# asalimil/Nonlinear-MPC-for-collision-free-and-deadlock-free-navigation-of-multiple-nonholonomic-mobile-robots

Hardware: AMD Instinct MI355X
Metric: NMPC solves/sec (batched swarms), N_robots=6, N=20 (higher is better)
Workload: dtype f64

## Files before the change

nonlinear-mpc-for-collision-free-and-deadlock-free-navigation-of-multiple-nonholonomic-mobile-robots_amd/csrc/nmpc_solve_col.hip:

```cpp
#include "nmpc_solve_common.h"

namespace nmpc {

__device__ __forceinline__ double lane_read(double v, int lane)
{
    return __hiloint2double(__builtin_amdgcn_readlane(__double2hiint(v), lane), __builtin_amdgcn_readlane(__double2loint(v), lane));
}
#ifndef NMPC_COL_GB
#define NMPC_COL_GB ((M_ == 6) ? (NX + 2) / 2 : NX + 1)
#endif
#ifndef NMPC_FW_PD
#define NMPC_FW_PD ((M_ <= 6) ? 2 : 1)
#endif
#ifndef NMPC_FW_FAKE
#define NMPC_FW_FAKE 0
#endif
#ifndef NMPC_COL_DPP
#define NMPC_COL_DPP 1
#endif
#ifndef NMPC_COL_WAVES_SMALL
#define NMPC_COL_WAVES_SMALL 1
#endif
#ifndef NMPC_COL_WAVES_MID
#define NMPC_COL_WAVES_MID 1
#endif
#ifndef NMPC_COL_WAVES_FOUR
#define NMPC_COL_WAVES_FOUR 2
#endif
#ifndef NMPC_COL_WAVES_LAT
#define NMPC_COL_WAVES_LAT 2
#endif
#ifndef NMPC_COL_DUMMY_ST
#define NMPC_COL_DUMMY_ST (NU - 1)
#endif
#ifndef NMPC_FUSE_DPHI
#define NMPC_FUSE_DPHI 1
#endif
#ifndef NMPC_COL_RP
#define NMPC_COL_RP 1
#endif

#define LC(c) (((c) < NU) ? NX + (c) : (c) - NU)

constexpr int rp_slot(int j) { return 2 * ((j >> 1) >> 1) + (j & 1); }
constexpr int rp_half(int j) { return (j >> 1) & 1; }
constexpr bool rp_live(int i, int jj, int nc, int nu) { return i >= nc || (4 * (i >> 1) + (i & 1) > jj) || (4 * (i >> 1) + 2 + (i & 1) > jj && 4 * (i >> 1) + 2 + (i & 1) < nu); }

constexpr int col_min_waves(int m, int thb, int dl)
{
    return m > 6 ? 1 : (m <= 3 ? NMPC_COL_WAVES_SMALL : (m == 4 ? NMPC_COL_WAVES_FOUR : ((m >= 5 && !thb && dl) ? NMPC_COL_WAVES_LAT : NMPC_COL_WAVES_MID)));
}

constexpr int NMPC_DL_OBS = 4;

typedef unsigned u32x2 __attribute__((ext_vector_type(2)));
template <int N_> __device__ __forceinline__ void fmac_rowb(double &acc, double u, double nr)
{
    asm("v_fmac_f64_dpp %0, %1, %2 row_newbcast:%3 row_mask:0xf bank_mask:0xf" : "+v"(acc) : "v"(u), "v"(nr), "n"(N_));
}
__device__ __forceinline__ void swap16(double &a, double &b)
{
    u32x2 lo = __builtin_amdgcn_permlane16_swap(__double2loint(a), __double2loint(b), false, false);
    u32x2 hi = __builtin_amdgcn_permlane16_swap(__double2hiint(a), __double2hiint(b), false, false);
    a = __hiloint2double(hi.x, lo.x); b = __hiloint2double(hi.y, lo.y);
}
__device__ __forceinline__ void swap32(double &a, double &b)
{
    u32x2 lo = __builtin_amdgcn_permlane32_swap(__double2loint(a), __double2loint(b), false, false);
    u32x2 hi = __builtin_amdgcn_permlane32_swap(__double2hiint(a), __double2hiint(b), false, false);
    a = __hiloint2double(hi.x, lo.x); b = __hiloint2double(hi.y, lo.y);
}

__device__ __forceinline__ double lane_gather(int src4, double v)
{
    return __hiloint2double(__builtin_amdgcn_ds_bpermute(src4, __double2hiint(v)), __builtin_amdgcn_ds_bpermute(src4, __double2loint(v)));
}

#ifndef NMPC_COL_SADDR
#define NMPC_COL_SADDR 1
#endif
struct UArr {
    double *b;
    int o;
    __device__ __forceinline__ double &operator[](int i) const
    {
#if NMPC_COL_SADDR
        return *reinterpret_cast<double *>(reinterpret_cast<char *>(b) + (size_t)((uint32_t)(o + i) * 8u));
#else
        return b[o + i];
#endif
    }
};

template <int M_, int THB> struct GC : G2<M_, THB> {
    using B = G2<M_, THB>;
    static constexpr int PK_CF = B::PK_CF;
    static constexpr int PK_T = PK_CF + 4 * M_;
    static constexpr int PK_ZERO = PK_T + 1;
    static constexpr int PACKC = ((PK_ZERO + 1 + 7) / 8) * 8;
    static constexpr int PACK = (PACKC < 64 && B::PACK >= 64) ? 64 : PACKC;
    static_assert(PACK <= B::PACK, "the workspace is sized for G2's pack");
};

template <int M_, int THB, int DL, int TPBK = 64>
__global__ __launch_bounds__(TPBK, col_min_waves(M_, THB, DL & 3)) void solve_col_kernel(const KParams P, const double *__restrict__ p_in, const double *__restrict__ w0,
                                                        double *__restrict__ w_out, double *__restrict__ obj_out,
                                                        int32_t *__restrict__ status_out, int32_t *__restrict__ iters_out,
                                                        double *__restrict__ kkt_out, double *__restrict__ ws, long long *__restrict__ prof_out)
{
    using G = GC<M_, THB>;
    constexpr int TPB = TPBK;
    static_assert(TPBK == 64 || TPBK == 128 || TPBK == 256, "one, two or four wavefronts per instance");
    constexpr int DLL = DL & 3;
    constexpr int NX = G::NX, NU = G::NU, NP = G::NP, NZ = G::NZ, LD = G::LD, NXB = G::NXB;
    constexpr int NPd = NP > 0 ? NP : 1;
    constexpr int MPN = M_ > 1 ? M_ - 1 : 1;
    static_assert(NZ <= 64, "one lane per column of the augmented matrix");
    constexpr int NR = (NZ + 15) / 16;
    constexpr bool RP = NMPC_COL_RP && M_ >= 2 && M_ <= 6;
    constexpr int MP = (M_ + 1) / 2, NC = 2 * MP, NS = 3 * MP, RR = NC + NS;
    const int tid = threadIdx.x;
    const int N = P.N, N1 = P.N + 1, K = P.K, MK = M_ * P.K;
    const double T = P.T;
    const size_t inst = (P.order && *P.order_bad == 0) ? (size_t)P.order[blockIdx.x] : (size_t)blockIdx.x;
    const ObsField<DL / NMPC_DL_OBS> OB(P, inst);
    double mu = P.mu_init;
    bool el = false;
    const bool prs = P.pairs != 0;
    const int NPA = prs ? G::NP : 0;

    extern __shared__ double sm[];
    double *X = sm;
    double *U = X + N1 * NX;
    double *LAM = U + N * NU;
    double *SN = LAM + N1 * NX;
    double *CS = SN + N * M_;
    double *DX = CS + N * M_;
    double *DU = DX + N1 * NX;
    double *RV = DU + N * NU;
    double *FS = RV, *PK = RV;
    constexpr int RG0 = G::KTS > G::PACK ? G::KTS : G::PACK;
    double *XS = RV + ((N1 * NX > RG0) ? N1 * NX : RG0);
    double *RED = XS + NX;
    double *gd = DLL ? (RED + 8) : (ws + inst * P.stride2 + P.oDUAL);
    const int oZPp = N1 * NP, oSO = oZPp + N1 * NP, oZO = oSO + N1 * MK, oZUL = oZO + N1 * MK, oZUU = oZUL + N * NU, oZXL = oZUU + N * NU, oZXU = oZXL + N1 * NXB,
              oSUL = oZXU + N1 * NXB, oSUU = oSUL + N * NU;
    const UArr SPp{gd, 0};
    const UArr ZPp{gd, oZPp};
    const UArr SO{gd, oSO};
    const UArr ZO{gd, oZO};
    const UArr ZUL{gd, oZUL};
    const UArr ZUU{gd, oZUU};
    const UArr ZXL{gd, oZXL};
    const UArr ZXU{gd, oZXU};
    const UArr SUL{gd, oSUL};
    const UArr SUU{gd, oSUU};

    double *const dl_end = DLL ? gd + oSUU + N * NU : RED + 8;
    double *gkt = (DLL >= 2) ? dl_end : ws + inst * P.stride2 + P.oKT;
    double *gpack = (DLL >= 3) ? dl_end + (size_t)N * G::KTS : ws + inst * P.stride2 + P.oPACK;
    const UArr TPp{ws + inst * P.stride2 + P.oELAS, 0};
    const UArr TOb{ws + inst * P.stride2 + P.oELAS, N1 * NP};
    const double rho = P.rho_el;
    double *gck = ws + inst * P.stride2 + P.oCKPT;
    const double *pp = p_in + inst * (2 * NX);
    const double *wi = w0 + inst * (size_t)P.nvar;
    double *wo = w_out + inst * (size_t)P.nvar;

#ifdef NMPC_POISON
    {
        const int nl = (int)((DLL ? gd + oSUU + N * NU : RED + 8) - sm) + (DLL >= 2 ? N * G::KTS : 0) + (DLL >= 3 ? N1 * G::PACK : 0);
        for (int e = tid; e < nl; e += TPB) sm[e] = NMPC_POISON;
        for (size_t e = tid; e < (size_t)P.stride2; e += TPB) ws[inst * P.stride2 + e] = NMPC_POISON;
        __syncthreads();
    }
#endif
#ifdef NMPC_PROFILE
    long long prof[12] = {0, 0, 0, 0, 0, 0, 0, 0, 0, 0, 0, 0};
    long long tlast = clock64();
#endif

    auto lbu = [&](int c) { return (c & 1) ? -P.wmax : -P.vmax; };
    auto bst = [&](int s) { return THB ? s : 3 * (s >> 1) + (s & 1); };
    auto bvl = [&](int s) { return (THB && (s % 3 == 2)) ? P.thmax : P.xymax; };

    const bool is_state = tid < NX, is_ctrl = tid >= NX && tid < NZ, lvalid = tid < NZ;
    const int ms = is_state ? tid : 0;
    const int ma = is_ctrl ? tid - NX : 0;
    const int mycol = is_state ? NU + ms : ma;
    const int mrob = is_state ? ms / 3 : ma >> 1;
    const bool th_lane = is_state && (ms - 3 * mrob == 2);
    const int srcA = 4 * (th_lane ? 3 * mrob : (is_ctrl ? ((ma & 1) ? 3 * mrob + 2 : 3 * mrob) : tid));
    const int srcB = 4 * (th_lane ? 3 * mrob + 1 : (is_ctrl ? ((ma & 1) ? 3 * mrob + 2 : 3 * mrob + 1) : tid));

    const double bp = 1e-2;
    for (int c = tid; c < NX; c += TPB) XS[c] = pp[NX + c];
    for (int e = tid; e < N1 * NX; e += TPB) {
        int k = e / NX, c = e - k * NX;
        double v = (k == 0) ? pp[c] : wi[e];
        if (k >= 1) {
            int d = c % 3;
            if (d < 2 || THB) {
                double b = (d == 2) ? P.thmax : P.xymax, px = fmin(bp * fmax(1.0, b), bp * 2.0 * b);
                v = fmin(fmax(v, -b + px), b - px);
            }
        }
        X[e] = v; LAM[e] = 0.0; DX[e] = 0.0;
    }
    for (int e = tid; e < N * NU; e += TPB) {
        int c = e % NU;
        double lo = lbu(c), hi = -lo, pu = fmin(bp * fmax(1.0, fabs(lo)), bp * (hi - lo));
        U[e] = fmin(fmax(wi[(size_t)N1 * NX + e], lo + pu), hi - pu);
        DU[e] = 0.0;
    }
    __syncthreads();

    {
        double bad = 0.0;
        for (int q = tid; q < NPA; q += TPB) {
            int i, j;
            pair_of<M_>(q, i, j);
            double dx = X[3 * i] - X[3 * j], dy = X[3 * i + 1] - X[3 * j + 1];
            if (h_pair(dx, dy, P.dmin2) < -NMPC_X0_TOL) bad = 1.0;
        }
        for (int e = tid; e < MK; e += TPB) {
            int i = e / K, o = e - i * K;
            double dx = X[3 * i] - OB(0, o, 0), dy = X[3 * i + 1] - OB(0, o, 1);
            if (h_obs(r_obs(dx, dy), P.robdim, OB(0, o, 2), P.margin) < -NMPC_X0_TOL) bad = 1.0;
        }
        bad = wmax<TPB>(bad, RED);
        if (bad > 0.0) {
            for (int e = tid; e < N1 * NX; e += TPB) wo[e] = X[e];
            for (int e = tid; e < N * NU; e += TPB) wo[(size_t)N1 * NX + e] = U[e];
            if (tid == 0) {
                if (obj_out) obj_out[inst] = NAN;
                if (status_out) status_out[inst] = NMPC_STATUS_INFEASIBLE_X0;
                if (iters_out) iters_out[inst] = 0;
                if (kkt_out) kkt_out[inst] = INFINITY;
            }
            return;
        }
    }

    auto pair_ij = [&](int q, int &i, int &j) { pair_of<M_>(q, i, j); };

    auto trig = [&]() {
        for (int it = tid; it < N * M_; it += TPB) {
            int k = it / M_, i = it - k * M_;
            double s, c;
            sincos(X[k * NX + 3 * i + 2], &s, &c);
            SN[it] = s; CS[it] = c;
        }
    };
    auto merit_t = [&](auto elc, double a, double &fv, double &lg, double &th, double &ec_, double &eh_) {
        constexpr bool EL = decltype(elc)::value;
        double fs = 0.0, t = 0.0, mc = 0.0, mh = 0.0;
        LogSum ls;
// ... 311 lines not shown
                            const int q = pidx_any<M_>(i, p + (p >= i ? 1 : 0));
                            sq[p] = SPp[k * NP + q]; zq[p] = ZPp[k * NP + q];
                        });
                        static_for<0, M_ - 1>([&](auto pc) {
                            constexpr int p = decltype(pc)::value;
                            const int j = p + (p >= i ? 1 : 0);
                            double dx = xi - x[3 * j], dy = yi - x[3 * j + 1];
                            double sv = sq[p], zv = zq[p], sg, v;
                            if constexpr (EL) el_sigma(mu, rho, sv, zv, TPp[k * NP + pidx_any<M_>(i, j)], h_pair(dx, dy, P.dmin2), sg, v);
                            else { sg = qdiv(zv, sv); v = qdiv(mu, sv) - sg * (h_pair(dx, dy, P.dmin2) - sv); }
                            g0 -= 2 * dx * v; g1 -= 2 * dy * v;
                            h0 += 4 * sg * dx * dx - 2 * zv; hxy += 4 * sg * dx * dy; h1 += 4 * sg * dy * dy - 2 * zv;
                        });
                    }
                    for (int o = 0; o < K; o++) {
                        double dx = xi - OB(k, o, 0), dy = yi - OB(k, o, 1), rr = r_obs(dx, dy), n0 = qdiv(dx, rr), n1 = qdiv(dy, rr);
                        double sv = SO[k * MK + i * K + o], zv = ZO[k * MK + i * K + o], sg, v, zz = qdiv(zv, rr);
                        if constexpr (EL) el_sigma(mu, rho, sv, zv, TOb[k * MK + i * K + o], h_obs(rr, P.robdim, OB(k, o, 2), P.margin), sg, v);
                        else { sg = qdiv(zv, sv); v = qdiv(mu, sv) - sg * (h_obs(rr, P.robdim, OB(k, o, 2), P.margin) - sv); }
                        g0 -= n0 * v; g1 -= n1 * v;
                        h0 += sg * n0 * n0 - zz * (1 - n0 * n0); hxy += sg * n0 * n1 + zz * n0 * n1; h1 += sg * n1 * n1 - zz * (1 - n1 * n1);
                    }
                }
            }
            double hvt = 0.0;
            if (k < N) {
                const double *u = U + k * NU + 2 * i, *ln = LAM + (k + 1) * NX + 3 * i;
                double c = CS[it], s = SN[it];
                if (k >= 1) h2 += T * u[0] * (ln[0] * c + ln[1] * s);
                hvt = T * (ln[0] * s - ln[1] * c);
#pragma unroll
                for (int d = 0; d < 2; d++) {
                    const int eu = k * NU + 2 * i + d;
                    double lo = d ? -P.wmax : -P.vmax, sl = SUL[eu], su = SUU[eu], zl = ZUL[eu], zu = ZUU[eu];
                    double vl = qdiv(mu, sl) - qdiv(zl, sl) * ((u[d] - lo) - sl), vu = qdiv(mu, su) - qdiv(zu, su) * ((-lo - u[d]) - su);
                    pk[G::PK_G + 2 * i + d] = 2 * P.r[d] * u[d] - (vl - vu);
                    pk[G::PK_HD + 2 * i + d] = 2 * P.r[d] + qdiv(zl, sl) + qdiv(zu, su);
                }
                {
                    double *cf = pk + G::PK_CF + 4 * i;
                    cf[0] = T * c; cf[1] = T * s; cf[2] = -T * u[0] * s; cf[3] = T * u[0] * c;
                }
                const double *xn = x + NX;
                pk[G::PK_C + 3 * i] = defect_xy(xn[3 * i], x[3 * i], T * u[0], c);
                pk[G::PK_C + 3 * i + 1] = defect_xy(xn[3 * i + 1], x[3 * i + 1], T * u[0], s);
                pk[G::PK_C + 3 * i + 2] = defect_th(xn[3 * i + 2], x[3 * i + 2], T, u[1]);
                pk[G::PK_HVT + i] = hvt;
            }
            pk[G::PK_G + NU + 3 * i] = g0; pk[G::PK_G + NU + 3 * i + 1] = g1; pk[G::PK_G + NU + 3 * i + 2] = g2;
            pk[G::PK_HD + NU + 3 * i] = h0; pk[G::PK_HD + NU + 3 * i + 1] = h1; pk[G::PK_HD + NU + 3 * i + 2] = h2;
            pk[G::PK_HXY + i] = hxy;
        }
        for (int it = tid; it < (N - 1) * NPA; it += TPB) {
            int k = 1 + it / NPd, q = it - (k - 1) * NP, i, j;
            pair_ij(q, i, j);
            double dx = X[k * NX + 3 * i] - X[k * NX + 3 * j], dy = X[k * NX + 3 * i + 1] - X[k * NX + 3 * j + 1];
            double zz = ZPp[k * NP + q], sg;
            if constexpr (EL) { double v_; el_sigma(mu, rho, SPp[k * NP + q], zz, TPp[k * NP + q], h_pair(dx, dy, P.dmin2), sg, v_); }
            else sg = qdiv(zz, SPp[k * NP + q]);
            double *pk = gpack + (size_t)k * G::PACK + G::PK_E + 3 * q;
            pk[0] = -(4 * sg * dx * dx - 2 * zz); pk[1] = -(4 * sg * dx * dy); pk[2] = -(4 * sg * dy * dy - 2 * zz);
        }
        };
        if (el) stage_packs(std::true_type{}); else stage_packs(std::false_type{});
        __syncthreads();
        PROF_T(2);

        double delta = need_shift ? fmax(1e-20, 0.25 * delta_last) : 0.0;
        int ntry = 0;
        bool ok;
        int kst = N - 1;
        for (;;) {
            ok = true;
            int kf = 0;
            if (TPBK == 64 || tid < 64) {
            constexpr int TPB = 64;
            if constexpr (RP) {
            const int rh = tid >> 5, rw = (tid >> 4) & 1, rn = tid & 15;
            const bool cc_ = rn < NC;
            const int cp = cc_ ? (rn >> 1) : (rn - NC) / 3, cd = cc_ ? (rn & 1) : (rn - NC) - 3 * cp, crob = 2 * cp + rw;
            const bool cvalid = rn < RR && crob < M_, c_state = cvalid && !cc_, c_ctrl = cvalid && cc_;
            const int rcol = cvalid ? (cc_ ? 2 * crob + cd : NU + 3 * crob + cd) : 0;
            auto rob_ok = [&](int p) { return (M_ % 2 == 0) || p < MP - 1 || rh == 0; };
            int hoff[RR];
            static_for<0, RR>([&](auto ic) {
                constexpr int i = decltype(ic)::value;
                constexpr bool au = i < NC;
                constexpr int p = au ? (i >> 1) : (i - NC) / 3, d = au ? (i & 1) : (i - NC) - 3 * p;
                const int rob = 2 * p + rh;
                const int a = au ? 2 * rob + d : NU + 3 * rob + d;
                int h = G::PK_ZERO;
                if constexpr (!au && d < 2) {
                    const int lo = rob < crob ? rob : crob, hi = rob < crob ? crob : rob;
                    const int pe = G::PK_E + 3 * (lo * (2 * M_ - lo - 1) / 2 + (hi - lo - 1)) + d + cd;
                    h = (c_state && cd < 2) ? ((rob == crob) ? G::PK_HXY + rob : pe) : h;
                }
                if constexpr (au && d == 0) h = (c_state && cd == 2 && crob == rob) ? G::PK_HVT + rob : h;
                if constexpr (!au && d == 2) h = (c_ctrl && cd == 0 && crob == rob) ? G::PK_HVT + rob : h;
                h = (rcol == a) ? G::PK_HD + a : h;
                hoff[i] = 8 * ((cvalid && rob < M_) ? h : G::PK_ZERO);
            });
            const int goff = 8 * (cvalid ? G::PK_G + rcol : G::PK_ZERO);
            const int cfA = 8 * ((c_state && cd == 2) ? G::PK_CF + 4 * crob + 2 : ((c_ctrl && cd == 0) ? G::PK_CF + 4 * crob : ((c_ctrl && cd == 1) ? G::PK_T : G::PK_ZERO)));
            const int cfB = 8 * ((c_state && cd == 2) ? G::PK_CF + 4 * crob + 3 : ((c_ctrl && cd == 0) ? G::PK_CF + 4 * crob + 1 : G::PK_ZERO));
            const int cbo = 8 * (G::PK_C + 3 * rh), cf1 = 8 * (G::PK_CF + 4 * rh);
            const int lb = tid & ~15;
            const bool needxy = (c_state && cd == 2) || (c_ctrl && cd == 0), needth = c_ctrl && cd == 1;
            const int srcA2 = 4 * (needxy ? lb + NC + 3 * cp : (needth ? lb + NC + 3 * cp + 2 : tid));
            const int srcB2 = 4 * (needxy ? lb + NC + 3 * cp + 1 : (needth ? lb + NC + 3 * cp + 2 : tid));
            double m[RR + 1];
            static_for<0, NC>([&](auto rc) { m[decltype(rc)::value] = 0.0; });
            if (kst == N - 1) {
                const double *pkN = gpack + (size_t)N * G::PACK;
                const double hdN = c_state ? pkN[G::PK_HD + rcol] : 0.0, gN = c_state ? pkN[G::PK_G + rcol] : 0.0;
                static_for<NC, RR>([&](auto rc) { constexpr int r = decltype(rc)::value; m[r] = (c_state && rw == rh && rn == r) ? hdN : 0.0; });
                m[RR] = gN;
            } else {
                const double *ck = gck + (size_t)((N - 1 - kst) / NMPC_CKPT_EVERY) * ((NX + 1) * 64) + tid;
                static_for<0, NS + 1>([&](auto rc) { constexpr int r = decltype(rc)::value; const double v = ck[r * 64]; m[NC + r] = cvalid ? v : 0.0; });
            }
            constexpr int PKR = (G::PACK + TPB - 1) / TPB;
            constexpr bool FULL = PKR * TPB <= RG0 && PKR * TPB <= 2 * G::PACK;
            double pkr[PKR];
#pragma unroll
            for (int t = 0; t < PKR; t++) { int e = tid + t * TPB; pkr[t] = (FULL || e < G::PACK) ? gpack[(size_t)kst * G::PACK + e] : 0.0; }
            double pend_row = 0.0, pend_rhs = 0.0;
            int ckc = 0;
#if NMPC_COL_DUMMY_ST
            static_for<0, NMPC_COL_DUMMY_ST>([&](auto jc) { gkt[(size_t)(N - 1) * G::KTS + decltype(jc)::value * G::LDC + NZ + 1] = 0.0; });
#endif
            for (int k = kst; k >= 0; k--) {
                lds_sync<TPB>();
#pragma unroll
                for (int t = 0; t < PKR; t++) {
                    const int e = tid + t * TPB;
                    if (FULL || e < G::PACK) PK[e] = (e >= G::PK_HD && e < G::PK_HD + NU) ? pkr[t] + delta : pkr[t];
                }
                if (k > 0) {
#pragma unroll
                    for (int t = 0; t < PKR; t++) { int e = tid + t * TPB; pkr[t] = (FULL || e < G::PACK) ? gpack[(size_t)(k - 1) * G::PACK + e] : 0.0; }
                }
                lds_sync<TPB>();
                double *const gkrow = gkt + (size_t)k * G::KTS + ((cvalid && rh == 0) ? rcol : NZ + 1);
                if (k < kst) {
                    gkrow[G::KTS + (NU - 1) * G::LDC] = pend_row;
                    if (tid < NU) gkt[(size_t)(k + 1) * G::KTS + tid * G::LDC + NZ] = pend_rhs;
                }
                if (ckc == NMPC_CKPT_EVERY) {
                    ckc = 0;
                    double *ck = gck + (size_t)((N - 1 - k) / NMPC_CKPT_EVERY) * ((NX + 1) * 64) + tid;
                    if (cvalid) static_for<0, NS + 1>([&](auto rc) { constexpr int r = decltype(rc)::value; ck[r * 64] = m[NC + r]; });
                }
                ckc++;
                double kO, kA, kB;
                {
                    kO = c_state ? 1.0 : 0.0; kA = lds_ld(PK, cfA, 0); kB = lds_ld(PK, cfB, 0);
                }
                {
                    double acc = 0.0;
                    static_for<0, NS>([&](auto sc) {
                        constexpr int s = decltype(sc)::value, p = s / 3, d = s - 3 * p;
                        double cv = lds_ld(PK, cbo, 8 * (6 * p + d));
                        if constexpr ((M_ & 1) && p == MP - 1) cv = rh ? 0.0 : cv;
                        acc = fma(m[NC + s], cv, acc);
                    });
                    double a2 = acc, b2 = acc;
                    swap32(a2, b2);
                    m[RR] -= a2 + b2;
                }
                {
#ifndef NMPC_RP_GB
#define NMPC_RP_GB (NS + 1)
#endif
                    constexpr int GB2 = NMPC_RP_GB;
                    static_for<0, (NS + 1 + GB2 - 1) / GB2>([&](auto bc) {
                        constexpr int q0 = decltype(bc)::value * GB2, q1 = (q0 + GB2 < NS + 1) ? q0 + GB2 : NS + 1;
                        double tA[GB2], tB[GB2];
                        static_for<q0, q1>([&](auto rc) { constexpr int q = decltype(rc)::value; tA[q - q0] = lane_gather(srcA2, m[NC + q]); tB[q - q0] = lane_gather(srcB2, m[NC + q]); });
                        static_for<q0, q1>([&](auto rc) { constexpr int q = decltype(rc)::value; m[NC + q] = fma(kB, tB[q - q0], fma(kA, tA[q - q0], kO * m[NC + q])); });
                    });
                }
                PROF_T(9);
                static_for<0, MP>([&](auto pc) {
                    constexpr int p = decltype(pc)::value;
                    double Tc = lds_ld(PK, cf1, 8 * (8 * p)), Ts = lds_ld(PK, cf1, 8 * (8 * p + 1)), Tt = T;
                    double ai = lds_ld(PK, cf1, 8 * (8 * p + 2)), bi = lds_ld(PK, cf1, 8 * (8 * p + 3));
                    if constexpr ((M_ & 1) && p == MP - 1) { Tc = rh ? 0.0 : Tc; Ts = rh ? 0.0 : Ts; Tt = rh ? 0.0 : Tt; ai = rh ? 0.0 : ai; bi = rh ? 0.0 : bi; }
                    const double gx = m[NC + 3 * p], gy = m[NC + 3 * p + 1], gt = m[NC + 3 * p + 2];
                    m[2 * p] = fma(Ts, gy, Tc * gx);
                    m[2 * p + 1] = Tt * gt;
                    m[NC + 3 * p + 2] = fma(bi, gy, fma(ai, gx, gt));
                });
                static_for<0, RR>([&](auto rc) { constexpr int r = decltype(rc)::value; m[r] += lds_ld(PK, hoff[r], 0); });
                m[RR] += lds_ld(PK, goff, 0);
                PROF_T(10);
                double thr = 0.0;
                static_for<0, NC>([&](auto ic) { constexpr int i = decltype(ic)::value; thr = (rh == rw && rn == i) ? m[i] : thr; });
                thr = 1e-9 * fabs(thr);
                auto pivot_inv = [&](double d) { return (d > thr) ? rcp_nr(d) : -1.0; };
                double inv_cur = lane_read(pivot_inv(m[rp_slot(0)]), 48 * rp_half(0) + rp_slot(0));
                double rhsv = 0.0;
                bool okk = true;
                static_for<0, NU>([&](auto jc) {
                    constexpr int j = decltype(jc)::value, hj = rp_half(j), ij = rp_slot(j);
                    const double inv = inv_cur;
                    okk = okk && (inv > 0.0);
                    const double rhs_j = lane_read(m[RR], 16 * hj + ij);
                    rhsv = (tid == j) ? -rhs_j * inv : rhsv;
                    double own = m[ij];
                    if constexpr (hj == 0) swap32(own, m[ij]); else swap32(m[ij], own);
                    const double rjv = own * inv;
                    double nrjv = -rjv;
                    {
                        int mc = rcol;
                        asm("" : "+v"(mc));
                        if constexpr (j == NU - 1) pend_row = (mc > j) ? nrjv : 0.0;
                        else gkrow[j * G::LDC] = (mc > j) ? nrjv : 0.0;
                    }
                    double ur = own, ub = own;
                    swap16(ur, ub);
                    swap32(ur, ub);
                    asm("s_nop 1" : "+v"(ur));
                    auto elim = [&](auto ac) { constexpr int i = decltype(ac)::value; fmac_rowb<i>(m[i], ur, nrjv); };
                    if constexpr (j + 1 < NU) {
                        elim(std::integral_constant<int, rp_slot(j + 1)>{});
                        inv_cur = lane_read(pivot_inv(m[rp_slot(j + 1)]), 48 * rp_half(j + 1) + rp_slot(j + 1));
                    }
                    static_for<0, RR>([&](auto ac) {
                        constexpr int i = decltype(ac)::value;
                        if constexpr (rp_live(i, j, NC, NU) && !(j + 1 < NU && i == rp_slot(j + 1))) elim(ac);
                    });
                    m[RR] = fma(-rhs_j, rjv, m[RR]);
                });
                ok = okk;
                PROF_T(11);
                if (!ok) { kf = k; break; }
                pend_rhs = rhsv;
                if (k == 0) {
                    gkrow[(NU - 1) * G::LDC] = pend_row;
                    if (tid < NU) gkt[tid * G::LDC + NZ] = pend_rhs;
                }
            }
            } else {
            int hoff[NZ];
            static_for<0, NZ>([&](auto ac) {
                constexpr int a = decltype(ac)::value;
                constexpr bool au = a < NU;
                constexpr int sa = au ? 0 : a - NU, ia = au ? (a >> 1) : sa / 3, da = sa - 3 * (sa / 3);
                int h = G::PK_ZERO;
                if constexpr (!au && da < 2) {
                    const int dc = ms - 3 * mrob;
                    const int lo = ia < mrob ? ia : mrob, hi = ia < mrob ? mrob : ia;
                    const int pe = G::PK_E + 3 * (lo * (2 * M_ - lo - 1) / 2 + (hi - lo - 1)) + da + dc;
                    h = (is_state && dc < 2) ? ((ia == mrob) ? G::PK_HXY + ia : pe) : h;
                }
                if constexpr (au && (a & 1) == 0) h = (is_state && ms == 3 * ia + 2) ? G::PK_HVT + ia : h;
                if constexpr (!au && da == 2) h = (is_ctrl && ma == 2 * ia) ? G::PK_HVT + ia : h;
                h = (lvalid && mycol == a) ? G::PK_HD + a : h;
                hoff[a] = 8 * (lvalid ? h : G::PK_ZERO);
            });
            const int goff = 8 * (lvalid ? G::PK_G + mycol : G::PK_ZERO);
            const int cfA = 8 * (th_lane ? G::PK_CF + 4 * mrob + 2 : ((is_ctrl && !(ma & 1)) ? G::PK_CF + 4 * mrob : ((is_ctrl && (ma & 1)) ? G::PK_T : G::PK_ZERO)));
            const int cfB = 8 * (th_lane ? G::PK_CF + 4 * mrob + 3 : ((is_ctrl && !(ma & 1)) ? G::PK_CF + 4 * mrob + 1 : G::PK_ZERO));
            double m[NZ + 1];
            static_for<0, NU>([&](auto rc) { m[decltype(rc)::value] = 0.0; });
            if (kst == N - 1) {
                const double *pkN = gpack + (size_t)N * G::PACK;
                const double hdN = is_state ? pkN[G::PK_HD + NU + ms] : 0.0, gN = is_state ? pkN[G::PK_G + NU + ms] : 0.0;
                static_for<0, NX>([&](auto rc) { constexpr int r = decltype(rc)::value; m[NU + r] = (is_state && ms == r) ? hdN : 0.0; });
                m[NZ] = gN;
            } else {
                const double *ck = gck + (size_t)((N - 1 - kst) / NMPC_CKPT_EVERY) * ((NX + 1) * 64) + tid;
                static_for<0, NX + 1>([&](auto rc) { constexpr int r = decltype(rc)::value; const double v = ck[r * 64]; m[NU + r] = is_state ? v : 0.0; });
            }
            constexpr int PKR = (G::PACK + TPB - 1) / TPB;
            constexpr bool FULL = PKR * TPB <= RG0 && PKR * TPB <= 2 * G::PACK;
            double pkr[PKR];
#pragma unroll
            for (int t = 0; t < PKR; t++) { int e = tid + t * TPB; pkr[t] = (FULL || e < G::PACK) ? gpack[(size_t)kst * G::PACK + e] : 0.0; }
            double pend_row = 0.0, pend_rhs = 0.0;
            int ckc = 0;
#if NMPC_COL_DUMMY_ST
            static_for<0, NMPC_COL_DUMMY_ST>([&](auto jc) { gkt[(size_t)(N - 1) * G::KTS + decltype(jc)::value * G::LDC + NZ + 1] = 0.0; });
#endif
            for (int k = kst; k >= 0; k--) {
                lds_sync<TPB>();
#pragma unroll
                for (int t = 0; t < PKR; t++) {
                    const int e = tid + t * TPB;
                    if (FULL || e < G::PACK) PK[e] = (e >= G::PK_HD && e < G::PK_HD + NU) ? pkr[t] + delta : pkr[t];
                }
                if (k > 0) {
#pragma unroll
                    for (int t = 0; t < PKR; t++) { int e = tid + t * TPB; pkr[t] = (FULL || e < G::PACK) ? gpack[(size_t)(k - 1) * G::PACK + e] : 0.0; }
                }
                lds_sync<TPB>();
                double *const gkrow = gkt + (size_t)k * G::KTS + (lvalid ? mycol : NZ + 1);
                if (k < kst) {
                    gkrow[G::KTS + (NU - 1) * G::LDC] = pend_row;
                    if (tid < NU) gkt[(size_t)(k + 1) * G::KTS + tid * G::LDC + NZ] = pend_rhs;
                }
                if (ckc == NMPC_CKPT_EVERY) {
                    ckc = 0;
                    double *ck = gck + (size_t)((N - 1 - k) / NMPC_CKPT_EVERY) * ((NX + 1) * 64) + tid;
                    if (is_state) static_for<0, NX + 1>([&](auto rc) { constexpr int r = decltype(rc)::value; ck[r * 64] = m[NU + r]; });
                }
                ckc++;
                double kO, kA, kB;
                {
                    kO = is_state ? 1.0 : 0.0; kA = lds_ld(PK, cfA, 0); kB = lds_ld(PK, cfB, 0);
                }
                static_for<0, NX>([&](auto sc) { constexpr int s = decltype(sc)::value; m[NZ] = fma(-m[NU + s], PK[G::PK_C + s], m[NZ]); });
                {
                    constexpr int GB = NMPC_COL_GB;
                    static_for<0, (NX + 1 + GB - 1) / GB>([&](auto bc) {
                        constexpr int q0 = decltype(bc)::value * GB, q1 = (q0 + GB < NX + 1) ? q0 + GB : NX + 1;
                        double tA[GB], tB[GB];
                        static_for<q0, q1>([&](auto rc) { constexpr int q = decltype(rc)::value; tA[q - q0] = lane_gather(srcA, m[NU + q]); tB[q - q0] = lane_gather(srcB, m[NU + q]); });
                        static_for<q0, q1>([&](auto rc) { constexpr int q = decltype(rc)::value; m[NU + q] = fma(kB, tB[q - q0], fma(kA, tA[q - q0], kO * m[NU + q])); });
                    });
                }
                PROF_T(9);
                static_for<0, M_>([&](auto ic) {
                    constexpr int i = decltype(ic)::value;
                    const double Tc = PK[G::PK_CF + 4 * i], Ts = PK[G::PK_CF + 4 * i + 1], Tt = T;
                    const double ai = PK[G::PK_CF + 4 * i + 2], bi = PK[G::PK_CF + 4 * i + 3];
                    const double gx = m[NU + 3 * i], gy = m[NU + 3 * i + 1], gt = m[NU + 3 * i + 2];
                    m[2 * i] = fma(Ts, gy, Tc * gx);
                    m[2 * i + 1] = Tt * gt;
                    m[NU + 3 * i + 2] = fma(bi, gy, fma(ai, gx, gt));
                });
                static_for<0, NZ>([&](auto rc) { constexpr int r = decltype(rc)::value; m[r] += lds_ld(PK, hoff[r], 0); });
                m[NZ] += lds_ld(PK, goff, 0);
                PROF_T(10);
                double d0s[NU];
                static_for<0, NU>([&](auto jc) { constexpr int j = decltype(jc)::value; d0s[j] = lane_read(m[j], LC(j)); });
                auto pivot_inv = [&](double d, double d0) { return (d > 1e-9 * fabs(d0)) ? rcp_nr(d) : -1.0; };
                double inv_cur = pivot_inv(d0s[0], d0s[0]);
                double rhsv = 0.0;
                bool okk = true;
                static_for<0, NU>([&](auto jc) {
                    constexpr int j = decltype(jc)::value;
                    {
                        const double inv = inv_cur;
                        okk = okk && (inv > 0.0);
                        {
                            const double rhs_j = lane_read(m[NZ], LC(j));
                            rhsv = (tid == j) ? -rhs_j * inv : rhsv;
                            const double rjv = m[j] * inv;
                            double nrjv = -rjv;
                            {
                                int mc = mycol;
                                asm("" : "+v"(mc));
                                if constexpr (j == NU - 1) pend_row = (mc > j) ? nrjv : 0.0;
                                else gkrow[j * G::LDC] = (mc > j) ? nrjv : 0.0;
                            }
#if NMPC_COL_DPP
                            double ur[NR < 3 ? NR : 4];
                            if constexpr (NR == 1) asm("s_nop 1" : "+v"(m[j]));
                            ur[0] = m[j];
                            if constexpr (NR == 2) { ur[1] = m[j]; swap16(ur[0], ur[1]); }
                            if constexpr (NR >= 3) {
                                ur[1] = m[j]; swap16(ur[0], ur[1]);
                                ur[2] = ur[0]; swap32(ur[0], ur[2]);
                                ur[3] = ur[1]; swap32(ur[1], ur[3]);
                            }
                            if constexpr (NR == 2) asm("s_nop 1" : "+v"(ur[0]), "+v"(ur[1]));
                            if constexpr (NR >= 3) asm("s_nop 1" : "+v"(ur[0]), "+v"(ur[1]), "+v"(ur[2]), "+v"(ur[3]));
                            auto elim = [&](auto ac) {
                                constexpr int a = decltype(ac)::value;
                                fmac_rowb<(LC(a) & 15)>(m[a], ur[LC(a) >> 4], nrjv);
                            };
#else
                            auto elim = [&](auto ac) {
                                constexpr int a = decltype(ac)::value;
                                m[a] = fma(-lane_read(m[j], LC(a)), rjv, m[a]);
                            };
#endif
                            if constexpr (j + 1 < NU) {
                                elim(std::integral_constant<int, j + 1>{});
                                inv_cur = pivot_inv(lane_read(m[j + 1], LC(j + 1)), d0s[j + 1]);
                            }
                            static_for<(j + 1 < NU ? j + 2 : j + 1), NZ>([&](auto ac) { elim(ac); });
                            m[NZ] = fma(-rhs_j, rjv, m[NZ]);
                        }
                    }
                });
                ok = okk;
                PROF_T(11);
                if (!ok) { kf = k; break; }
                pend_rhs = rhsv;
                if (k == 0) {
                    gkrow[(NU - 1) * G::LDC] = pend_row;
                    if (tid < NU) gkt[tid * G::LDC + NZ] = pend_rhs;
                }
            }
            }
            }
            if constexpr (TPBK > 64) {
                if (tid == 0) RED[7] = ok ? 1.0 : 0.0;
                __syncthreads();
                ok = __builtin_amdgcn_readfirstlane(RED[7] != 0.0 ? 1 : 0) != 0;
                __syncthreads();
            }
            if (ok) break;
            ntry++;
            if (delta == 0.0) delta = (delta_last == 0.0) ? 1e-4 : fmax(1e-20, delta_last / 3.0);
            else delta *= (delta_last == 0.0) ? 100.0 : NMPC_SHIFT_ESCALATION;
            if (delta > 1e20) break;
            kst = NMPC_RESUME_STAGE(kf, N);
        }
        if (!ok) { if (n_cold < NMPC_COLD_RETRIES) { cold_retry(); iter++; } else status = NMPC_STATUS_NUMERIC; break; }
        if (delta > 0.0) delta_last = delta;
        need_shift = delta > 0.0 && (ntry > 0 || delta > 1e-6);
        __syncthreads();
        PROF_T(3);

        if (TPBK == 64 || tid < 64) {
        constexpr int TPB = 64;
        if constexpr (NU <= 32 && NX <= 32) {
            constexpr int LDC = G::LDC, CT = (NX + 3) & ~1, CH = CT / 2, PD = NMPC_FW_PD;
            static_assert(NU + CT <= LDC && NU <= CT, "row chunks of the forward sweep");
            constexpr int TB = (NU <= 16) ? 16 : 0, BB = TB + 32;
            const bool isT = tid >= TB && tid < TB + NU, isB = tid >= BB && tid < BB + NU;
            const double2 *rowp = reinterpret_cast<const double2 *>(gkt + (isT ? (tid - TB) * LDC + NU : (isB ? (tid - BB) * LDC : NU)));
            double kq[PD][CT];
#pragma unroll
            for (int d = 0; d < PD; d++)
#pragma unroll
                for (int t = 0; t < CT; t++) kq[d][t] = 0.0;
            auto fetch = [&](auto dc, int k) {
                constexpr int d = decltype(dc)::value;
#pragma unroll
                for (int t = 0; t < CH; t++) {
                    const double2 v = rowp[(size_t)(NMPC_FW_FAKE ? 0 : k) * (G::KTS / 2) + t];
                    kq[d][2 * t] = v.x; kq[d][2 * t + 1] = v.y;
                }
            };
            static_for<0, PD>([&](auto dc) { if (decltype(dc)::value < N) fetch(dc, decltype(dc)::value); });
            double dx = 0.0;
            if (is_state) DX[tid] = 0.0;
            for (int k0 = 0; k0 < N; k0 += PD) {
                static_for<0, PD>([&](auto dc) {
                    constexpr int d = decltype(dc)::value;
                    const int k = k0 + d;
                    if (k < N) {
                        int ln = tid;
                        asm volatile("" : "+v"(ln));
                        const int fr = ln < NX ? ln : 0, fi = fr / 3, fd = fr - 3 * fi;
                        const int srcT = 4 * (3 * fi + 2), srcU = 4 * (BB + (fd < 2 ? 2 * fi : 2 * fi + 1));
                        const double sn = SN[k * M_ + fi], cs = CS[k * M_ + fi], uv = U[k * NU + 2 * fi], uw = U[k * NU + 2 * fi + 1];
                        const double xk = X[k * NX + fr], xn = X[(k + 1) * NX + fr];
                        const double dxt = lane_gather(srcT, dx);
                        double u0 = dx, u1 = dx;
                        swap16(u0, u1);
                        asm("s_nop 1" : "+v"(u0));
                        if constexpr (NX > 16) asm("s_nop 0" : "+v"(u1));
                        double t = kq[d][NX];
                        static_for<0, NX>([&](auto cc) {
                            constexpr int c = decltype(cc)::value;
                            if constexpr (c < 16) fmac_rowb<(c & 15)>(t, u0, kq[d][c]);
                            else fmac_rowb<(c & 15)>(t, u1, kq[d][c]);
                        });
                        double tb = t, tl = t;
                        swap32(tb, tl);
                        static_for<1, NU>([&](auto cc) {
                            constexpr int c = NU - decltype(cc)::value;
                            if constexpr (c < 16) {
                                asm("s_nop 1" : "+v"(tb));
                                double ub = tb;
                                fmac_rowb<c>(tb, ub, kq[d][c]);
                            } else {
                                tb = fma(kq[d][c], lane_read(tb, BB + c), tb);
                            }
                        });
                        if (ln >= BB && ln < BB + NU) DU[k * NU + (ln - BB)] = tb;
                        const double du = lane_gather(srcU, tb);
                        if (k + PD < N) fetch(dc, k + PD);
// ... 614 lines not shown
```

Before: 275,400.

## Micro-optimize column Riccati elimination: absolute LDS addressing, masked stores, scalar pivot checks

Bakes the LDS base into per-lane offsets so pack loads use absolute addresses. Pivot acceptance moves to scalar compare and ballot logic, and the rhs update becomes an exec-masked negated multiply instead of a select. Gain-row stores are redirected through compile-time lane masks to a dummy column instead of storing selected zeros, with a one-time zero-fill of the lower triangle and padding at kernel start. The goal is fewer VALU selects and address computations in the hot per-stage loop, in exchange for inline asm fragility and an extra initialization pass.

```diff
diff --git a/nonlinear-mpc-for-collision-free-and-deadlock-free-navigation-of-multiple-nonholonomic-mobile-robots_amd/csrc/nmpc_solve_col.hip b/nonlinear-mpc-for-collision-free-and-deadlock-free-navigation-of-multiple-nonholonomic-mobile-robots_amd/csrc/nmpc_solve_col.hip
--- a/nonlinear-mpc-for-collision-free-and-deadlock-free-navigation-of-multiple-nonholonomic-mobile-robots_amd/csrc/nmpc_solve_col.hip
+++ b/nonlinear-mpc-for-collision-free-and-deadlock-free-navigation-of-multiple-nonholonomic-mobile-robots_amd/csrc/nmpc_solve_col.hip
@@ -1,6 +1,28 @@
 #include "nmpc_solve_common.h"
 
 namespace nmpc {
+
+typedef __attribute__((address_space(3))) const double lds_cdouble;
+__device__ __forceinline__ int lds_addr(const double *p) { return (int)(unsigned)(size_t)(lds_cdouble *)p; }
+__device__ __forceinline__ double lds_ld_abs(int addr, int cbytes) { return *(lds_cdouble *)(size_t)(unsigned)(addr + cbytes); }
+
+__device__ __forceinline__ bool sgpr_positive(int hi)
+{
+    int f;
+    asm("s_sub_u32 %0, %1, 1\n\ts_cmp_lt_u32 %0, 0x7fefffff\n\ts_cselect_b32 %0, 1, 0" : "=s"(f) : "s"(hi) : "scc");
+    return f != 0;
+}
+
+__device__ __forceinline__ int lane_const(int v)
+{
+    asm("" : "+v"(v));
+    return v;
+}
+#ifndef NMPC_COL_LDSB
+#define NMPC_COL_LDSB 1
+#endif
+template <bool ABS = (NMPC_COL_LDSB != 0)> __device__ __forceinline__ int pk_off(int pkb, int off) { return ABS ? lane_const(pkb + off) : off; }
+template <bool ABS = (NMPC_COL_LDSB != 0)> __device__ __forceinline__ double pk_ld(const double *PK, int off, int cbytes) { return ABS ? lds_ld_abs(off, cbytes) : lds_ld(PK, off, cbytes); }
 
 __device__ __forceinline__ double lane_read(double v, int lane)
 {
@@ -38,6 +60,18 @@
 #endif
 #ifndef NMPC_COL_RP
 #define NMPC_COL_RP 1
+#endif
+#ifndef NMPC_COL_SPIV
+#define NMPC_COL_SPIV 1
+#endif
+#ifndef NMPC_COL_MST
+#define NMPC_COL_MST 1
+#endif
+#ifndef NMPC_COL_RHSL
+#define NMPC_COL_RHSL 1
+#endif
+#ifndef NMPC_COL_BK_LAT
+#define NMPC_COL_BK_LAT 0
 #endif
 
 #define LC(c) (((c) < NU) ? NX + (c) : (c) - NU)
@@ -45,6 +79,36 @@
 constexpr int rp_slot(int j) { return 2 * ((j >> 1) >> 1) + (j & 1); }
 constexpr int rp_half(int j) { return (j >> 1) & 1; }
 constexpr bool rp_live(int i, int jj, int nc, int nu) { return i >= nc || (4 * (i >> 1) + (i & 1) > jj) || (4 * (i >> 1) + 2 + (i & 1) > jj && 4 * (i >> 1) + 2 + (i & 1) < nu); }
+constexpr unsigned long long rp_store_mask(int m, int j, bool ctrl_only = false)
+{
+    const int mp = (m + 1) / 2, nc = 2 * mp, rr = 5 * mp, nu = 2 * m;
+    unsigned long long msk = 0;
+    for (int t = 0; t < 32; t++) {
+        const int rw = t >> 4, rn = t & 15;
+        const bool cc = rn < nc;
+        const int cp = cc ? (rn >> 1) : (rn - nc) / 3, cd = cc ? (rn & 1) : (rn - nc) - 3 * cp, crob = 2 * cp + rw;
+        const int rcol = cc ? 2 * crob + cd : nu + 3 * crob + cd;
+        if (rn < rr && crob < m && rcol > j && (cc || !ctrl_only)) msk |= 1ull << t;
+    }
+    return msk;
+}
+constexpr unsigned long long col_store_mask(int m, int j)
+{
+    unsigned long long msk = 0;
+    for (int t = 0; t < 5 * m; t++)
+        if ((t < 3 * m ? 2 * m + t : t - 3 * m) > j) msk |= 1ull << t;
+    return msk;
+}
+__device__ __forceinline__ void neg_mul_lanes(double &dst, double a, double s, unsigned long long msk)
+{
+    unsigned long long sv;
+    asm("s_and_saveexec_b64 %1, %4\n\tv_mul_f64 %0, -%2, %3\n\ts_mov_b64 exec, %1" : "+v"(dst), "=&s"(sv) : "v"(a), "s"(s), "s"(msk) : "scc");
+}
+__device__ __forceinline__ void neg_mul_lanes_v(double &dst, double a, double s, unsigned long long msk)
+{
+    unsigned long long sv;
+    asm("s_and_saveexec_b64 %1, %4\n\tv_mul_f64 %0, -%2, %3\n\ts_mov_b64 exec, %1" : "+v"(dst), "=&s"(sv) : "v"(a), "v"(s), "s"(msk) : "scc");
+}
 
 constexpr int col_min_waves(int m, int thb, int dl)
 {
@@ -173,6 +237,16 @@
         for (int e = tid; e < nl; e += TPB) sm[e] = NMPC_POISON;
         for (size_t e = tid; e < (size_t)P.stride2; e += TPB) ws[inst * P.stride2 + e] = NMPC_POISON;
         __syncthreads();
+    }
+#endif
+#if NMPC_COL_MST
+    if constexpr (!RP || TPBK == 64 || NMPC_COL_BK_LAT) {
+        for (int e = tid; e < N * NU; e += TPB) {
+            const int k = e / NU, j = e - k * NU;
+            double *row = gkt + (size_t)k * G::KTS + j * G::LDC;
+            for (int c = 0; c <= j; c++) row[c] = 0.0;
+            for (int c = NZ + 1; c < G::LDC; c++) row[c] = 0.0;
+        }
     }
 #endif
 #ifdef NMPC_PROFILE
@@ -650,6 +724,9 @@
             const bool cvalid = rn < RR && crob < M_, c_state = cvalid && !cc_, c_ctrl = cvalid && cc_;
             const int rcol = cvalid ? (cc_ ? 2 * crob + cd : NU + 3 * crob + cd) : 0;
             auto rob_ok = [&](int p) { return (M_ % 2 == 0) || p < MP - 1 || rh == 0; };
+            constexpr bool BK_ = TPBK == 64 || NMPC_COL_BK_LAT;
+            constexpr bool SPIV_ = NMPC_COL_SPIV && BK_, MST_ = NMPC_COL_MST && BK_, RHSL_ = NMPC_COL_RHSL && BK_, LDSB_ = NMPC_COL_LDSB && BK_;
+            const int pkb = lds_addr(PK);
             int hoff[RR];
             static_for<0, RR>([&](auto ic) {
                 constexpr int i = decltype(ic)::value;
@@ -666,12 +743,13 @@
                 if constexpr (au && d == 0) h = (c_state && cd == 2 && crob == rob) ? G::PK_HVT + rob : h;
                 if constexpr (!au && d == 2) h = (c_ctrl && cd == 0 && crob == rob) ? G::PK_HVT + rob : h;
                 h = (rcol == a) ? G::PK_HD + a : h;
-                hoff[i] = 8 * ((cvalid && rob < M_) ? h : G::PK_ZERO);
+                hoff[i] = pk_off<LDSB_>(pkb, 8 * ((cvalid && rob < M_) ? h : G::PK_ZERO));
             });
-            const int goff = 8 * (cvalid ? G::PK_G + rcol : G::PK_ZERO);
-            const int cfA = 8 * ((c_state && cd == 2) ? G::PK_CF + 4 * crob + 2 : ((c_ctrl && cd == 0) ? G::PK_CF + 4 * crob : ((c_ctrl && cd == 1) ? G::PK_T : G::PK_ZERO)));
-            const int cfB = 8 * ((c_state && cd == 2) ? G::PK_CF + 4 * crob + 3 : ((c_ctrl && cd == 0) ? G::PK_CF + 4 * crob + 1 : G::PK_ZERO));
-            const int cbo = 8 * (G::PK_C + 3 * rh), cf1 = 8 * (G::PK_CF + 4 * rh);
+            const int goff = pk_off<LDSB_>(pkb, 8 * (cvalid ? G::PK_G + rcol : G::PK_ZERO));
+            const int rco8 = 8 * rcol;
+            const int cfA = pk_off<LDSB_>(pkb, 8 * ((c_state && cd == 2) ? G::PK_CF + 4 * crob + 2 : ((c_ctrl && cd == 0) ? G::PK_CF + 4 * crob : ((c_ctrl && cd == 1) ? G::PK_T : G::PK_ZERO))));
+            const int cfB = pk_off<LDSB_>(pkb, 8 * ((c_state && cd == 2) ? G::PK_CF + 4 * crob + 3 : ((c_ctrl && cd == 0) ? G::PK_CF + 4 * crob + 1 : G::PK_ZERO)));
+            const int cbo = pk_off<LDSB_>(pkb, 8 * (G::PK_C + 3 * rh)), cf1 = pk_off<LDSB_>(pkb, 8 * (G::PK_CF + 4 * rh));
             const int lb = tid & ~15;
             const bool needxy = (c_state && cd == 2) || (c_ctrl && cd == 0), needth = c_ctrl && cd == 1;
             const int srcA2 = 4 * (needxy ? lb + NC + 3 * cp : (needth ? lb + NC + 3 * cp + 2 : tid));
@@ -710,10 +788,21 @@
                 }
                 lds_sync<TPB>();
                 double *const gkrow = gkt + (size_t)k * G::KTS + ((cvalid && rh == 0) ? rcol : NZ + 1);
-                if (k < kst) {
-                    gkrow[G::KTS + (NU - 1) * G::LDC] = pend_row;
-                    if (tid < NU) gkt[(size_t)(k + 1) * G::KTS + tid * G::LDC + NZ] = pend_rhs;
-                }
+                auto st_row = [&](auto jc, int kk, double v) {
+                    constexpr int j = decltype(jc)::value;
+                    if constexpr (MST_) {
+                    int so = __builtin_amdgcn_inverse_ballot_w64(rp_store_mask(M_, j)) ? rco8 : 8 * (NZ + 1);
+                    asm("" : "+v"(so));
+                    reinterpret_cast<double *>(reinterpret_cast<char *>(gkt + (size_t)kk * G::KTS) + (size_t)(uint32_t)so)[j * G::LDC] = v;
+                    } else
+                    gkrow[(size_t)(kk - k) * G::KTS + j * G::LDC] = v;
+                };
+                auto st_pend = [&](int kk) {
+                    st_row(std::integral_constant<int, NU - 1>{}, kk, pend_row);
+                    if constexpr (RHSL_) { if (__builtin_amdgcn_inverse_ballot_w64(rp_store_mask(M_, -1, true))) gkt[(size_t)kk * G::KTS + rcol * G::LDC + NZ] = pend_rhs; }
+                    else { if (tid < NU) gkt[(size_t)kk * G::KTS + tid * G::LDC + NZ] = pend_rhs; }
+                };
+                if (k < kst) st_pend(k + 1);
                 if (ckc == NMPC_CKPT_EVERY) {
                     ckc = 0;
                     double *ck = gck + (size_t)((N - 1 - k) / NMPC_CKPT_EVERY) * ((NX + 1) * 64) + tid;
@@ -722,13 +811,13 @@
                 ckc++;
                 double kO, kA, kB;
                 {
-                    kO = c_state ? 1.0 : 0.0; kA = lds_ld(PK, cfA, 0); kB = lds_ld(PK, cfB, 0);
+                    kO = c_state ? 1.0 : 0.0; kA = pk_ld<LDSB_>(PK, cfA, 0); kB = pk_ld<LDSB_>(PK, cfB, 0);
                 }
                 {
                     double acc = 0.0;
                     static_for<0, NS>([&](auto sc) {
                         constexpr int s = decltype(sc)::value, p = s / 3, d = s - 3 * p;
-                        double cv = lds_ld(PK, cbo, 8 * (6 * p + d));
+                        double cv = pk_ld<LDSB_>(PK, cbo, 8 * (6 * p + d));
                         if constexpr ((M_ & 1) && p == MP - 1) cv = rh ? 0.0 : cv;
                         acc = fma(m[NC + s], cv, acc);
                     });
@@ -751,39 +840,52 @@
                 PROF_T(9);
                 static_for<0, MP>([&](auto pc) {
                     constexpr int p = decltype(pc)::value;
-                    double Tc = lds_ld(PK, cf1, 8 * (8 * p)), Ts = lds_ld(PK, cf1, 8 * (8 * p + 1)), Tt = T;
-                    double ai = lds_ld(PK, cf1, 8 * (8 * p + 2)), bi = lds_ld(PK, cf1, 8 * (8 * p + 3));
+                    double Tc = pk_ld<LDSB_>(PK, cf1, 8 * (8 * p)), Ts = pk_ld<LDSB_>(PK, cf1, 8 * (8 * p + 1)), Tt = T;
+                    double ai = pk_ld<LDSB_>(PK, cf1, 8 * (8 * p + 2)), bi = pk_ld<LDSB_>(PK, cf1, 8 * (8 * p + 3));
                     if constexpr ((M_ & 1) && p == MP - 1) { Tc = rh ? 0.0 : Tc; Ts = rh ? 0.0 : Ts; Tt = rh ? 0.0 : Tt; ai = rh ? 0.0 : ai; bi = rh ? 0.0 : bi; }
                     const double gx = m[NC + 3 * p], gy = m[NC + 3 * p + 1], gt = m[NC + 3 * p + 2];
                     m[2 * p] = fma(Ts, gy, Tc * gx);
                     m[2 * p + 1] = Tt * gt;
                     m[NC + 3 * p + 2] = fma(bi, gy, fma(ai, gx, gt));
                 });
-                static_for<0, RR>([&](auto rc) { constexpr int r = decltype(rc)::value; m[r] += lds_ld(PK, hoff[r], 0); });
-                m[RR] += lds_ld(PK, goff, 0);
+                static_for<0, RR>([&](auto rc) { constexpr int r = decltype(rc)::value; m[r] += pk_ld<LDSB_>(PK, hoff[r], 0); });
+                m[RR] += pk_ld<LDSB_>(PK, goff, 0);
                 PROF_T(10);
                 double thr = 0.0;
                 static_for<0, NC>([&](auto ic) { constexpr int i = decltype(ic)::value; thr = (rh == rw && rn == i) ? m[i] : thr; });
                 thr = 1e-9 * fabs(thr);
-                auto pivot_inv = [&](double d) { return (d > thr) ? rcp_nr(d) : -1.0; };
-                double inv_cur = lane_read(pivot_inv(m[rp_slot(0)]), 48 * rp_half(0) + rp_slot(0));
+                bool acc_cur = true;
+                auto pivot_inv = [&](double d, auto lc) {
+                    constexpr int L = decltype(lc)::value;
+                    if constexpr (SPIV_) {
+                        const double r = lane_read(rcp_nr(d), L);
+                        acc_cur = (((__builtin_amdgcn_fcmp(d, thr, 2 ) >> L) & 1) != 0) & sgpr_positive(__double2hiint(r));
+                        return r;
+                    } else
+                        return lane_read((d > thr) ? rcp_nr(d) : -1.0, L);
+                };
+                double inv_cur = pivot_inv(m[rp_slot(0)], std::integral_constant<int, 48 * rp_half(0) + rp_slot(0)>{});
                 double rhsv = 0.0;
                 bool okk = true;
                 static_for<0, NU>([&](auto jc) {
                     constexpr int j = decltype(jc)::value, hj = rp_half(j), ij = rp_slot(j);
                     const double inv = inv_cur;
-                    okk = okk && (inv > 0.0);
+                    if constexpr (SPIV_) okk = okk && acc_cur; else okk = okk && (inv > 0.0);
                     const double rhs_j = lane_read(m[RR], 16 * hj + ij);
-                    rhsv = (tid == j) ? -rhs_j * inv : rhsv;
+                    if constexpr (RHSL_) neg_mul_lanes(rhsv, m[RR], inv, 1ull << (16 * hj + ij));
+                    else rhsv = (tid == j) ? -rhs_j * inv : rhsv;
                     double own = m[ij];
                     if constexpr (hj == 0) swap32(own, m[ij]); else swap32(m[ij], own);
                     const double rjv = own * inv;
                     double nrjv = -rjv;
-                    {
+                    if constexpr (MST_) {
+                        if constexpr (j == NU - 1) pend_row = nrjv;
+                        else st_row(jc, k, nrjv);
+                    } else {
                         int mc = rcol;
                         asm("" : "+v"(mc));
                         if constexpr (j == NU - 1) pend_row = (mc > j) ? nrjv : 0.0;
-                        else gkrow[j * G::LDC] = (mc > j) ? nrjv : 0.0;
+                        else st_row(jc, k, (mc > j) ? nrjv : 0.0);
                     }
                     double ur = own, ub = own;
                     swap16(ur, ub);
@@ -792,7 +894,7 @@
                     auto elim = [&](auto ac) { constexpr int i = decltype(ac)::value; fmac_rowb<i>(m[i], ur, nrjv); };
                     if constexpr (j + 1 < NU) {
                         elim(std::integral_constant<int, rp_slot(j + 1)>{});
-                        inv_cur = lane_read(pivot_inv(m[rp_slot(j + 1)]), 48 * rp_half(j + 1) + rp_slot(j + 1));
+                        inv_cur = pivot_inv(m[rp_slot(j + 1)], std::integral_constant<int, 48 * rp_half(j + 1) + rp_slot(j + 1)>{});
                     }
                     static_for<0, RR>([&](auto ac) {
                         constexpr int i = decltype(ac)::value;
@@ -804,12 +906,10 @@
                 PROF_T(11);
                 if (!ok) { kf = k; break; }
                 pend_rhs = rhsv;
-                if (k == 0) {
-                    gkrow[(NU - 1) * G::LDC] = pend_row;
-                    if (tid < NU) gkt[tid * G::LDC + NZ] = pend_rhs;
-                }
+                if (k == 0) st_pend(0);
             }
             } else {
+            const int pkb = lds_addr(PK);
             int hoff[NZ];
             static_for<0, NZ>([&](auto ac) {
                 constexpr int a = decltype(ac)::value;
@@ -825,11 +925,12 @@
                 if constexpr (au && (a & 1) == 0) h = (is_state && ms == 3 * ia + 2) ? G::PK_HVT + ia : h;
                 if constexpr (!au && da == 2) h = (is_ctrl && ma == 2 * ia) ? G::PK_HVT + ia : h;
                 h = (lvalid && mycol == a) ? G::PK_HD + a : h;
-                hoff[a] = 8 * (lvalid ? h : G::PK_ZERO);
+                hoff[a] = pk_off(pkb, 8 * (lvalid ? h : G::PK_ZERO));
             });
-            const int goff = 8 * (lvalid ? G::PK_G + mycol : G::PK_ZERO);
-            const int cfA = 8 * (th_lane ? G::PK_CF + 4 * mrob + 2 : ((is_ctrl && !(ma & 1)) ? G::PK_CF + 4 * mrob : ((is_ctrl && (ma & 1)) ? G::PK_T : G::PK_ZERO)));
-            const int cfB = 8 * (th_lane ? G::PK_CF + 4 * mrob + 3 : ((is_ctrl && !(ma & 1)) ? G::PK_CF + 4 * mrob + 1 : G::PK_ZERO));
+            const int goff = pk_off(pkb, 8 * (lvalid ? G::PK_G + mycol : G::PK_ZERO));
+            const int mco8 = 8 * mycol;
+            const int cfA = pk_off(pkb, 8 * (th_lane ? G::PK_CF + 4 * mrob + 2 : ((is_ctrl && !(ma & 1)) ? G::PK_CF + 4 * mrob : ((is_ctrl && (ma & 1)) ? G::PK_T : G::PK_ZERO))));
+            const int cfB = pk_off(pkb, 8 * (th_lane ? G::PK_CF + 4 * mrob + 3 : ((is_ctrl && !(ma & 1)) ? G::PK_CF + 4 * mrob + 1 : G::PK_ZERO)));
             double m[NZ + 1];
             static_for<0, NU>([&](auto rc) { m[decltype(rc)::value] = 0.0; });
             if (kst == N - 1) {
@@ -864,10 +965,25 @@
                 }
                 lds_sync<TPB>();
                 double *const gkrow = gkt + (size_t)k * G::KTS + (lvalid ? mycol : NZ + 1);
-                if (k < kst) {
-                    gkrow[G::KTS + (NU - 1) * G::LDC] = pend_row;
-                    if (tid < NU) gkt[(size_t)(k + 1) * G::KTS + tid * G::LDC + NZ] = pend_rhs;
-                }
+                auto st_row = [&](auto jc, int kk, double v) {
+                    constexpr int j = decltype(jc)::value;
+#if NMPC_COL_MST
+                    int so = __builtin_amdgcn_inverse_ballot_w64(col_store_mask(M_, j)) ? mco8 : 8 * (NZ + 1);
+                    asm("" : "+v"(so));
+                    reinterpret_cast<double *>(reinterpret_cast<char *>(gkt + (size_t)kk * G::KTS) + (size_t)(uint32_t)so)[j * G::LDC] = v;
+#else
+                    gkrow[(size_t)(kk - k) * G::KTS + j * G::LDC] = v;
+#endif
+                };
+                auto st_pend = [&](int kk) {
+                    st_row(std::integral_constant<int, NU - 1>{}, kk, pend_row);
+#if NMPC_COL_RHSL
+                    if (is_ctrl) gkt[(size_t)kk * G::KTS + ma * G::LDC + NZ] = pend_rhs;
+#else
+                    if (tid < NU) gkt[(size_t)kk * G::KTS + tid * G::LDC + NZ] = pend_rhs;
+#endif
+                };
+                if (k < kst) st_pend(k + 1);
                 if (ckc == NMPC_CKPT_EVERY) {
                     ckc = 0;
                     double *ck = gck + (size_t)((N - 1 - k) / NMPC_CKPT_EVERY) * ((NX + 1) * 64) + tid;
@@ -876,7 +992,7 @@
                 ckc++;
                 double kO, kA, kB;
                 {
-                    kO = is_state ? 1.0 : 0.0; kA = lds_ld(PK, cfA, 0); kB = lds_ld(PK, cfB, 0);
+                    kO = is_state ? 1.0 : 0.0; kA = pk_ld(PK, cfA, 0); kB = pk_ld(PK, cfB, 0);
                 }
                 static_for<0, NX>([&](auto sc) { constexpr int s = decltype(sc)::value; m[NZ] = fma(-m[NU + s], PK[G::PK_C + s], m[NZ]); });
                 {
@@ -898,12 +1014,17 @@
                     m[2 * i + 1] = Tt * gt;
                     m[NU + 3 * i + 2] = fma(bi, gy, fma(ai, gx, gt));
                 });
-                static_for<0, NZ>([&](auto rc) { constexpr int r = decltype(rc)::value; m[r] += lds_ld(PK, hoff[r], 0); });
-                m[NZ] += lds_ld(PK, goff, 0);
+                static_for<0, NZ>([&](auto rc) { constexpr int r = decltype(rc)::value; m[r] += pk_ld(PK, hoff[r], 0); });
+                m[NZ] += pk_ld(PK, goff, 0);
                 PROF_T(10);
                 double d0s[NU];
                 static_for<0, NU>([&](auto jc) { constexpr int j = decltype(jc)::value; d0s[j] = lane_read(m[j], LC(j)); });
+#if NMPC_COL_SPIV
+                bool acc_cur;
+                auto pivot_inv = [&](double d, double d0) { const double r = rcp_nr(d); acc_cur = d > 1e-9 * fabs(d0) && r > 0.0; return r; };
+#else
                 auto pivot_inv = [&](double d, double d0) { return (d > 1e-9 * fabs(d0)) ? rcp_nr(d) : -1.0; };
+#endif
                 double inv_cur = pivot_inv(d0s[0], d0s[0]);
                 double rhsv = 0.0;
                 bool okk = true;
@@ -911,17 +1032,30 @@
                     constexpr int j = decltype(jc)::value;
                     {
                         const double inv = inv_cur;
+#if NMPC_COL_SPIV
+                        okk = okk && acc_cur;
+#else
                         okk = okk && (inv > 0.0);
+#endif
                         {
                             const double rhs_j = lane_read(m[NZ], LC(j));
+#if NMPC_COL_RHSL
+                            neg_mul_lanes_v(rhsv, m[NZ], inv, 1ull << LC(j));
+#else
                             rhsv = (tid == j) ? -rhs_j * inv : rhsv;
+#endif
                             const double rjv = m[j] * inv;
                             double nrjv = -rjv;
                             {
+#if NMPC_COL_MST
+                                if constexpr (j == NU - 1) pend_row = nrjv;
+                                else st_row(jc, k, nrjv);
+#else
                                 int mc = mycol;
                                 asm("" : "+v"(mc));
                                 if constexpr (j == NU - 1) pend_row = (mc > j) ? nrjv : 0.0;
-                                else gkrow[j * G::LDC] = (mc > j) ? nrjv : 0.0;
+                                else st_row(jc, k, (mc > j) ? nrjv : 0.0);
+#endif
                             }
 #if NMPC_COL_DPP
                             double ur[NR < 3 ? NR : 4];
@@ -958,10 +1092,7 @@
                 PROF_T(11);
                 if (!ok) { kf = k; break; }
                 pend_rhs = rhsv;
-                if (k == 0) {
-                    gkrow[(NU - 1) * G::LDC] = pend_row;
-                    if (tid < NU) gkt[tid * G::LDC + NZ] = pend_rhs;
-                }
+                if (k == 0) st_pend(0);
             }
             }
             }
```

Result: faster. 285,900 (median of 6 runs) (+3.8%).
